# nasa/atmospheric-neural-rendering

Hardware: AMD Instinct MI355X
Metric: train-step rays/sec (higher is better)
Workload: dtype f16; 1 GPU; instant_ngp BASELINE configs[2]: 16-level T=2^19 hash grid, 2x64 fused MLP, 1024 samples/ray, full train step (fwd+loss+bwd+AdamW); global_batch=8192, per_rank_batch=8192, samples_per_ray=1024, parallelism=dp1

## Files before the change

### atmospheric-neural-rendering_amd/atmonr_amd/_lib.py

```python

from __future__ import annotations

import ctypes
import os
from ctypes import (
    POINTER,
    Structure,
    c_double,
    c_float,
    c_int32,
    c_int64,
    c_uint32,
    c_void_p,
)

import torch

_HERE = os.path.dirname(os.path.abspath(__file__))
LIB_PATH = os.environ.get("ANR_HIP_LIB", os.path.join(_HERE, "_native", "libanr_hip.so"))

F32, F16, BF16 = 0, 1, 2
MAX_LEVELS = 32

LOSS_CODES = {
# ... 240 lines not shown
         _P, _P, _P, c_int64, _P, c_int64, _P, _P, _P, c_int64, _P],
    ),
    "anr_occupancy_n_blocks": (c_int64, [c_int64]),
    "anr_occupancy_count": (
        c_int32, [_P, c_int64, _P, c_int32, c_int32, c_int32, c_float, _P, _P]),
    "anr_occupancy_compact": (
        c_int32, [_P, c_int64, _P, c_int32, c_int32, c_int32, c_float, _P, _P, _P, _P]),
    "anr_composite_force_generic": (c_int32, [c_int32]),
    "anr_composite_fwd": (
        c_int32,
        [_P, c_float, _P, _P, _P, c_int32, c_int64, c_int32, c_int32, c_int32,
         _P, _P, _P, _P, _P, _P],
    ),
    "anr_composite_bwd": (
        c_int32,
        [_P, c_float, _P, _P, _P, c_int32, c_int64, c_int32, c_int32, c_int32,
         _P, _P, _P, _P, _P, _P, _P, _P, _P, _P],
    ),
    "anr_loss_workspace_bytes": (c_int64, [c_int64]),
    "anr_loss_fwd_bwd": (
        c_int32,
        [c_int32, _P, c_int32, c_int32, _P, _P, c_int64, c_float, c_float, _P, _P, _P, _P],
    ),
    "anr_composite_ref16_set_rays": (c_int32, [c_int32]),
    "anr_composite_ref16_fwd": (
        c_int32,
        [_P, c_float, _P, _P, _P, c_int32, c_int64, c_int32, c_int32, _P, _P, _P, _P, _P, _P,
         _P, _P],
    ),
    "anr_composite_ref16_bwd": (
        c_int32,
        [_P, c_float, _P, _P, _P, c_int32, c_int64, c_int32, c_int32, _P, _P, _P, _P, c_int32,
         _P, _P],
    ),
    "anr_loss_ref16_fwd_bwd": (
        c_int32, [c_int32, _P, c_int32, _P, _P, c_int64, c_float, _P, _P, _P, _P]),
    "anr_grad_quantize_f16": (c_int32, [_P, c_int64, c_float, _P]),
    "anr_ingp_field_bwd_ref16": (
        c_int32,
        [POINTER(MlpDesc), POINTER(MlpDesc), _P, _P, c_int64, _P, c_int64, c_int64, _P, _P,
         c_int64, _P, c_int64, _P, _P, c_float, _P],
    ),
    "anr_ingp_field_bwd_ref16_tiles": (
        c_int32,
        [POINTER(MlpDesc), POINTER(MlpDesc), _P, _P, c_int64, _P, c_int64, c_int64, _P, _P,
         c_int64, _P, c_int64, _P, _P, c_float, _P, _P],
    ),
    "anr_ingp_field_bwd_ref16_rows": (
        c_int32,
        [POINTER(MlpDesc), POINTER(MlpDesc), _P, _P, c_int64, _P, c_int64, c_int64, _P, _P,
         c_int64, _P, c_int64, _P, _P, c_float, _P, _P, c_int64, _P],
    ),
    "anr_ingp_field_bwd_ref16_rows_h": (
        c_int32,
        [POINTER(MlpDesc), POINTER(MlpDesc), _P, _P, c_int64, _P, c_int64, c_int64, _P, _P,
         c_int64, _P, c_int64, _P, _P, c_float, _P, _P, c_int64, _P],
    ),
    "anr_ingp_field_bwd_ref16_rows_workspace_bytes": (c_int64, [c_int64]),
    "anr_mlp_bwd_ref16": (
        c_int32,
        [POINTER(MlpDesc), _P, _P, c_int32, c_int64, c_int64, _P, c_int32, c_int64, _P,
         c_int32, c_int64, _P, _P, c_int64, c_float, _P],
    ),
    "anr_adam_step": (
        c_int32,
        [_P, _P, _P, _P, _P, c_int64, c_float, c_float, c_float, c_float, c_float,
# ... 253 lines not shown
```

### atmospheric-neural-rendering_amd/atmonr_amd/graphics_utils.py

```python

from __future__ import annotations

import torch

from . import _lib
from ._lib import ANRError, call, dtype_code, ptr


class _CompositeFn(torch.autograd.Function):
    @staticmethod
    def forward(ctx, z, color, sigma, color_surf, z_scale: float, want_alpha: bool):
        B, N, C = color.shape
        S = sigma.shape[2]
        dt = color.dtype
        dev = color.device
        sigma = sigma.to(dt).contiguous()
        color = color.contiguous()
        cs = color_surf.to(dt).contiguous() if color_surf is not None else None
        zc = z.float().contiguous()
        color_map = torch.empty(B, C, device=dev, dtype=dt)
        atmo = torch.empty(B, C, device=dev, dtype=dt) if cs is not None else None
        surf = torch.empty(B, C, device=dev, dtype=dt) if cs is not None else None
        weights = torch.empty(B, N, S, device=dev, dtype=dt)
        alpha = torch.empty(B, N, S, device=dev, dtype=dt)
# ... 15 lines not shown
        B, N, C = color.shape
        S = sigma.shape[2]
        dt = color.dtype
        dev = color.device
        if ctx.has_surf:
            g_cm, g_alpha, g_w, g_atmo, g_surf = grads
        else:
            g_cm, g_alpha, g_w = grads
            g_atmo = g_surf = None

        def prep(g):
            return None if g is None else g.to(dt).contiguous()

        if g_cm is None:
            g_cm = torch.zeros(B, color.shape[2], device=dev, dtype=dt)

        need_z, need_c, need_s, need_cs = ctx.needs_input_grad[:4]
        d_color = torch.empty_like(color) if need_c else None
        d_sigma = torch.empty_like(sigma) if need_s else None
        d_cs = torch.empty_like(cs) if (need_cs and cs is not None) else None
        d_z = torch.empty(B, N, device=dev, dtype=torch.float32) if need_z else None
        args = (ptr(zc), ctx.z_scale, ptr(color), ptr(sigma), ptr(cs), dtype_code(dt), B, N, C,
                S, ptr(prep(g_cm)), ptr(prep(g_atmo)), ptr(prep(g_surf)), ptr(prep(g_w)),
                ptr(prep(g_alpha)), ptr(d_color), ptr(d_sigma), ptr(d_cs), ptr(d_z))
        call("anr_composite_bwd", *args, _lib.stream(dev))
        if d_z is not None:
            d_z = d_z.to(ctx.z_dtype)
        return d_z, d_color, d_sigma, d_cs, None, None


class _CompositeRef16Fn(torch.autograd.Function):

    @staticmethod
    def forward(ctx, z, color, sigma, color_surf, z_scale: float, zero_rays, want16: bool):
        B, N, C = color.shape
        if sigma.shape[2] != 1:
            raise ANRError("reference-numerics composite: one density channel (B, N, 1)")
        dev = color.device
        color, sigma = color.contiguous(), sigma.contiguous()
        cs = color_surf.to(color.dtype).contiguous() if color_surf is not None else None
        zc = z.float().contiguous()
        f16 = torch.float16
        cm = torch.empty(B, C, device=dev, dtype=f16)
        atmo = torch.empty(B, C, device=dev, dtype=f16)
        surf = torch.empty(B, C, device=dev, dtype=f16) if cs is not None else None
        weights = torch.empty(B, N, 1, device=dev, dtype=f16)
        alpha = torch.empty(B, N, 1, device=dev, dtype=f16)
        copies = want16 and color.dtype != f16
        c16 = torch.empty(B, N, C, device=dev, dtype=f16) if copies else None
        s16 = torch.empty(B, N, 1, device=dev, dtype=f16) if copies else None
        call("anr_composite_ref16_fwd", ptr(zc), float(z_scale), ptr(color), ptr(sigma), ptr(cs),
             dtype_code(color.dtype), B, N, C, ptr(cm), ptr(atmo), ptr(surf), ptr(weights),
             ptr(alpha), ptr(c16), ptr(s16), _lib.stream(dev), tag="composite_fwd")
        ctx.out_dtype = color.dtype
        if copies:
            ctx.save_for_backward(zc, c16, s16, cs)
        else:
            ctx.save_for_backward(zc, color, sigma, cs)
            if want16:
                c16, s16 = color.detach(), sigma.detach()
        ctx.set_materialize_grads(False)
        ctx.z_scale = float(z_scale)
        ctx.zero_rays = zero_rays
        outs = (cm, alpha, weights) if cs is None else (cm, alpha, weights, atmo, surf)
        if want16:
            ctx.mark_non_differentiable(c16, s16)
            outs = outs + (c16, s16)
        return outs

    @staticmethod
    def backward(ctx, g_cm, *unused):
        zc, color, sigma, cs = ctx.saved_tensors
        if any(g is not None for g in unused):
            raise ANRError("reference-numerics composite: gradients flow through color_map "
                           "only (as in the reference's loss)")
        B, N, C = color.shape
        dev = color.device
        if g_cm is None:
            g_cm = torch.zeros(B, C, device=dev, dtype=torch.float16)
        g_cm = g_cm.to(torch.float16).contiguous()
        od = ctx.out_dtype
        d_color = torch.empty(color.shape, device=dev, dtype=od)
        d_sigma = torch.empty(sigma.shape, device=dev, dtype=od)
        d_cs = (torch.empty(cs.shape, device=dev, dtype=od)
                if cs is not None and ctx.needs_input_grad[3] else None)
        if cs is not None and cs.dtype != color.dtype:
            cs = cs.to(color.dtype)
        call("anr_composite_ref16_bwd", ptr(zc), ctx.z_scale, ptr(color), ptr(sigma), ptr(cs),
             dtype_code(color.dtype), B, N, C, ptr(g_cm), ptr(d_color), ptr(d_sigma), ptr(d_cs),
             dtype_code(od), ptr(ctx.zero_rays), _lib.stream(dev), tag="composite_bwd")
        return None, d_color, d_sigma, d_cs, None, None, None


def render_with_surface_ref16(z_vals, color, sigma, color_surf, z_scale: float = 1.0,
                              zero_rays: torch.Tensor | None = None, inputs_f16: bool = False):
    _check(z_vals, color, sigma)
    if zero_rays is None:
        zero_rays = torch.zeros(1, dtype=torch.int32, device=color.device)
    return _CompositeRef16Fn.apply(z_vals, color, sigma, color_surf, z_scale, zero_rays,
                                   bool(inputs_f16))


def _check(z_vals, color, sigma):
    if not (z_vals.dim() == 2 and color.dim() == 3 and sigma.dim() == 3):
        raise ANRError("render: expected z (B,N), color (B,N,C), sigma (B,N,S)")
    if z_vals.shape != color.shape[:2] or z_vals.shape != sigma.shape[:2]:
        raise ANRError("render: z / color / sigma shapes disagree")
    if color.dtype not in (torch.float16, torch.float32):
        raise ANRError(f"render: unsupported dtype {color.dtype}")


def render(z_vals: torch.Tensor, color: torch.Tensor, sigma: torch.Tensor, z_scale: float = 1.0):
    _check(z_vals, color, sigma)
    return _CompositeFn.apply(z_vals, color, sigma, None, z_scale, True)


def render_with_surface(z_vals, color, sigma, color_surf, z_scale: float = 1.0):
    _check(z_vals, color, sigma)
    return _CompositeFn.apply(z_vals, color, sigma, color_surf, z_scale, True)
```

### atmospheric-neural-rendering_amd/atmonr_amd/pipelines/instant_ngp.py

```python

from __future__ import annotations

import os
from itertools import chain
from typing import Any, Mapping

import torch
import torch.nn.functional as F
from torch.optim import Optimizer

from .. import _lib
from ..field import IngpFieldFn, field_density, field_fused
from ..graphics_utils import render_with_surface, render_with_surface_ref16
from ..losses import LOSSES, indexed_loss, indexed_loss_ref16
from ..occupancy import OccupancyGrid, pipeline_density
from ..optim import FusedAdam
from ..samplers import (points_with_heights, preprocess_points, sample_and_preprocess,
                        sample_uniform_bins)
from ..tcnn import Encoding, Network
from .pipeline import Pipeline


class InstantNGPPipeline(Pipeline):
    module_names = ["pos_encoder", "pos_mlp", "dir_encoder", "dir_mlp", "surf_encoder",
# ... 139 lines not shown
                out = _lib.JoinAtBackwardEnd.apply(out, main)

        def join():
            main.wait_stream(side)
            out.record_stream(main)
            return out
        return join

    def _forward_fused(self, ray_batch, u=None):
        B = ray_batch["origin"].shape[0]
        N = self.config["num_samples_per_ray"]
        surf_branch = self._surface_async(ray_batch)
        _, z_vals, coords = sample_and_preprocess(ray_batch, N, self._prep_ngp, u=u)
        occ = self.occupancy
        if occ is not None and self.training:
            occ.update(pipeline_density(self))
        params = (self.pos_encoder.params, self.pos_mlp.params, self.dir_mlp.params, self)
        _lib.grad_use(*params[:3])
        if occ is not None and occ.active:
            rows, kept = occ.compact(coords.view(B * N, 3))
            sigma, color = IngpFieldFn.apply(kept, ray_batch["dir"].float(), N, *params, rows,
                                             B * N)
        else:
            sigma, color = IngpFieldFn.apply(coords.view(B * N, coords.shape[-1]),
                                             ray_batch["dir"].float(), N, *params)
        color = color.view(B, N, -1)
        sigma = sigma.view(B, N, 1)
        color_surf = surf_branch()
        if self.numerics == "reference":
            if self._zero_rays is None:
                self._zero_rays = torch.zeros(1, dtype=torch.int32, device=color.device)
            color_map, _, weights, atmo, surf, color, sigma = render_with_surface_ref16(
                z_vals, color, sigma, color_surf, z_scale=self.scale / 1000,
                zero_rays=self._zero_rays, inputs_f16=True)
            if color_map.requires_grad:
                color_map = _TcnnGradsAtBackwardEnd.apply(color_map, self)
        else:
            color_map, _, weights, atmo, surf = render_with_surface(
                z_vals, color, sigma, color_surf, z_scale=self.scale / 1000)
        results = {
            "color_fine": color[:, :-1],
            "color_surf": color_surf,
            "color_map_surf": surf,
            "color_map_atmo": atmo,
            "sigma_fine": sigma[:, :-1],
            "color_map_fine": color_map,
            "weights_fine": weights,
            "z_vals_fine": z_vals,
        }
        if self.include_height:
            results["norm_heights_fine"] = coords[..., 3]
        return results

    def _forward_reference(self, ray_batch, u=None):
        B_ = ray_batch["origin"].shape[0]
        N = self.config["num_samples_per_ray"]
        pts, z_vals = sample_uniform_bins(ray_batch, N, u=u)
        if self.point_preprocessor:
            pts = self.point_preprocessor(pts)
        pts = (pts + 1) / 2
        if self.include_height:
            pts = points_with_heights(pts, self._prep_height)
        dirs = ray_batch["dir"][:, None].repeat(1, N, 1)
        pts[..., 2] = pts[..., 2] / self.config["alt_compress_factor"]
        pos_enc = self.pos_encoder(pts.view(B_ * N, -1))
        pos_out = self.pos_mlp(pos_enc)
        dir_enc = self.dir_encoder(
# ... 108 lines not shown
```

### atmospheric-neural-rendering_amd/csrc/ref16.hip

```cpp
#pragma clang fp contract(off)

#include <stdlib.h>

#include <type_traits>

#include "anr_common.h"

namespace anr {
namespace ref16 {

constexpr int kMaxC = 8;
constexpr int kSeg = 64;

__device__ __forceinline__ float h(float x) {
  asm("" : "+v"(x));
  return __half2float(__float2half_rn(x));
}

__device__ __forceinline__ float h64(double d) {
  float f = static_cast<float>(d);
  if (static_cast<double>(f) != d && f != 0.0f && isfinite(f)) {
    uint32_t u = __float_as_uint(f);
    if (fabs(static_cast<double>(f)) > fabs(d)) u -= 1;
    f = __uint_as_float(u | 1u);
// ... 70 lines not shown
__device__ __forceinline__ Sample from_e(float e, float dl) {
  Sample s;
  s.delta = dl;
  s.e = e;
  s.alpha = h(1.0f - s.e);
  s.q2 = h(h(1.0f - s.alpha) + 1e-10f);
  return s;
}

__device__ __forceinline__ Sample sample(float sig, float dl) {
  const float x = h(-sig * dl);
  return from_e(h64(exp(static_cast<double>(x))), dl);
}

constexpr int kPad = 72;

template <int R>
struct __attribute__((aligned(16))) FwdLds {
  _Float16 q2[R][kPad];
  _Float16 alpha[R][kPad];
  _Float16 T[R][kPad];
  _Float16 t[kMaxC][R][kPad];
};
typedef _Float16 h8v __attribute__((ext_vector_type(8)));

__device__ __forceinline__ float mul_h(float a, _Float16 q) {
  return __builtin_fmaf(a, static_cast<float>(q), 0.0f);
}
__device__ __forceinline__ float add_h(float acc, _Float16 x) {
  return __builtin_fmaf(static_cast<float>(x), 1.0f, acc);
}
constexpr float kNegZero = -0.0f;

template <int R, typename T>
__global__ void __launch_bounds__(64) fwd_kernel(const float* __restrict__ z, float zs,
                                                 const T* __restrict__ color,
                                                 const T* __restrict__ sigma,
                                                 const T* __restrict__ cs, int64_t B, int N,
                                                 int C, __half* cmap, __half* atmo_out,
                                                 __half* surf_out, __half* weights,
                                                 __half* alpha_out, __half* color16,
                                                 __half* sigma16) {
  __shared__ FwdLds<R> L;
  const int64_t b0 = static_cast<int64_t>(blockIdx.x) * R;
  const int nr = B - b0 < R ? static_cast<int>(B - b0) : R;
  const int lane = threadIdx.x;
  const int sr = lane / C, sc = lane - sr * C;
  _Float16 cp = 1.0f;
  float pr = 1.0f;
  float acc = 0.0f;
  SegIn<R, true, true> nxt;
  nxt.fetch(z, sigma, color, b0, nr, 0, N, C, lane);
  for (int s0 = 0; s0 < N; s0 += kSeg) {
    const int n = N - s0 < kSeg ? N - s0 : kSeg;
    const int nv = (n + 7) & ~7;
    const SegIn<R, true, true> cur = nxt;
    if (s0 + kSeg < N) nxt.fetch(z, sigma, color, b0, nr, s0 + kSeg, N, C, lane);
#pragma unroll
    for (int r = 0; r < R; ++r) {
      if (r < nr && lane < n) {
        const int64_t b = b0 + r;
        const float sg = in16<T>(cur.sg[r]);
        if (sigma16) sigma16[b * N + s0 + lane] = __float2half_rn(sg);
        const Sample sm = sample(sg, delta_z(cur.zm[r], cur.z0[r], cur.zp[r], zs, s0 + lane, N));
        L.q2[r][lane] = static_cast<_Float16>(sm.q2);
        L.alpha[r][lane] = static_cast<_Float16>(sm.alpha);
      } else if (lane < nv) {
        L.q2[r][lane] = static_cast<_Float16>(1.0f);
      }
    }
    wave_sync();
    if (lane < nr) {
      for (int l8 = 0; l8 < nv; l8 += 8) {
        const h8v q = *reinterpret_cast<const h8v*>(&L.q2[lane][l8]);
        h8v tv;
#pragma unroll
        for (int k = 0; k < 8; ++k) {
          tv[k] = cp;
          cp = cp * q[k];
          pr = mul_h(pr, q[k]);
        }
        *reinterpret_cast<h8v*>(&L.T[lane][l8]) = tv;
      }
    }
    wave_sync();
#pragma unroll
    for (int r = 0; r < R; ++r) {
      if (r < nr && lane < n) {
        const int64_t i = (b0 + r) * N + s0 + lane;
        const float al = static_cast<float>(L.alpha[r][lane]);
        const float w = h(al * static_cast<float>(L.T[r][lane]));
#pragma unroll
        for (int c = 0; c < kMaxC; ++c) {
          if (c >= C) break;
          const float col = in16<T>(cur.col[r][c]);
          if (color16) color16[i * C + c] = __float2half_rn(col);
          L.t[c][r][lane] = static_cast<_Float16>(h(col * w));
        }
        if (weights) weights[i] = __float2half_rn(w);
        if (alpha_out) alpha_out[i] = __float2half_rn(al);
      } else if (lane < nv) {
        for (int c = 0; c < C; ++c) L.t[c][r][lane] = static_cast<_Float16>(kNegZero);
      }
    }
    wave_sync();
    if (sr < nr) {
      for (int l8 = 0; l8 < nv; l8 += 8) {
        const h8v tv = *reinterpret_cast<const h8v*>(&L.t[sc][sr][l8]);
#pragma unroll
        for (int k = 0; k < 8; ++k) acc = add_h(acc, tv[k]);
      }
    }
    wave_sync();
  }
  const float prr = h(__shfl(pr, sr < R ? sr : 0));
  if (sr < nr) {
    const int64_t b = b0 + sr;
    const int c = sc;
    const float atmo = h(acc);
    const float surf = cs ? h(prr * h(ld(cs, b * C + c))) : 0.0f;
    cmap[b * C + c] = __float2half_rn(cs ? h(atmo + surf) : atmo);
    if (atmo_out) atmo_out[b * C + c] = __float2half_rn(atmo);
    if (surf_out && cs) surf_out[b * C + c] = __float2half_rn(surf);
  }
}

template <int R>
struct __attribute__((aligned(16))) BwdLds {
  _Float16 q2[R][kPad];
  _Float16 u[R][kPad];
  _Float16 rin[R][kPad];
  float g[R][kMaxC];
  float g_pr[R];
  float pr[R];
};

template <int R, typename T, typename G>
__global__ void __launch_bounds__(64) bwd_kernel(const float* __restrict__ z, float zs,
                                                 const T* __restrict__ color,
                                                 const T* __restrict__ sigma,
                                                 const T* __restrict__ cs, int64_t B, int N,
                                                 int C, const __half* __restrict__ g_cm,
                                                 G* d_color, G* d_sigma, G* d_cs,
                                                 int* zero_rays) {
  __shared__ BwdLds<R> L;
  const int64_t b0 = static_cast<int64_t>(blockIdx.x) * R;
  const int nr = B - b0 < R ? static_cast<int>(B - b0) : R;
  const int lane = threadIdx.x;
  const int sr = lane / C, sc = lane - sr * C;
  constexpr bool GH = std::is_same<G, __half>::value;
  typedef uint32_t __attribute__((may_alias)) pair_t;
  const bool pair = GH && C >= 2 && ((static_cast<int64_t>(N) * C) & 1) == 0 &&
                    (reinterpret_cast<uintptr_t>(d_color) & 3) == 0;
  auto park = [&](int64_t b) { return reinterpret_cast<pair_t*>(d_color + b * N * C); };
  auto in = [](float x) {
    if constexpr (GH) return in16<T>(x);
    else return h(x);
  };
  const bool cvec = GH && color_vec4(color, C);
  float gl = 0.0f;
  if (sr < nr) {
    gl = __half2float(g_cm[(b0 + sr) * C + sc]);
    L.g[sr][sc] = gl;
  }
  _Float16 cp = 1.0f;
  float pr = 1.0f;
  uint32_t zmask = 0;
  SegIn<R, false, true> nxt;
  nxt.fetch(z, sigma, color, b0, nr, 0, N, C, lane);
  for (int s0 = 0; s0 < N; s0 += kSeg) {
    const int n = N - s0 < kSeg ? N - s0 : kSeg;
    const int nv = (n + 7) & ~7;
    const SegIn<R, false, true> cur = nxt;
    if (s0 + kSeg < N) nxt.fetch(z, sigma, color, b0, nr, s0 + kSeg, N, C, lane);
    float e1[R];
#pragma unroll
    for (int r = 0; r < R; ++r) {
      bool zr = false;
      e1[r] = 0.0f;
      if (r < nr && lane < n) {
        const int64_t b = b0 + r;
        const Sample sm = sample(in(cur.sg[r]),
                                 delta_z(cur.zm[r], cur.z0[r], cur.zp[r], zs, s0 + lane, N));
        L.q2[r][lane] = static_cast<_Float16>(sm.q2);
        e1[r] = sm.e;
        if (!(GH && pair)) d_color[(b * N + s0 + lane) * C] = static_cast<G>(sm.e);
        zr = sm.q2 == 0.0f;
      } else if (lane < nv) {
        L.q2[r][lane] = static_cast<_Float16>(1.0f);
      }
      if (__any(zr)) zmask |= 1u << r;
    }
    wave_sync();
    if (lane < nr) {
      for (int l8 = 0; l8 < nv; l8 += 8) {
        const h8v q = *reinterpret_cast<const h8v*>(&L.q2[lane][l8]);
        h8v tv;
#pragma unroll
        for (int k = 0; k < 8; ++k) {
          tv[k] = cp;
          cp = cp * q[k];
          pr = mul_h(pr, q[k]);
        }
        *reinterpret_cast<h8v*>(&L.u[lane][l8]) = tv;
      }
    }
    wave_sync();
#pragma unroll
    for (int r = 0; r < R; ++r)
      if (r < nr && lane < n) {
        if (GH && pair) {
          const uint32_t tb = __builtin_bit_cast(uint16_t, L.u[r][lane]);
          const uint32_t eb = __builtin_bit_cast(uint16_t, static_cast<_Float16>(e1[r]));
          park(b0 + r)[s0 + lane] = tb | (eb << 16);
        } else {
          d_sigma[(b0 + r) * N + s0 + lane] = static_cast<G>(static_cast<float>(L.u[r][lane]));
        }
      }
    wave_sync();
  }
  const float prr = h(__shfl(pr, sr < R ? sr : 0));
  if (lane < nr) L.pr[lane] = h(pr);
  if (cs && sr < nr) {
    if (d_cs) d_cs[(b0 + sr) * C + sc] = static_cast<G>(h(gl * prr));
  }
  if (lane < nr) {
    float g_pr = 0.0f;
    if (cs) {
      for (int c = 0; c < C; ++c) {
        const float csv = h(ld(cs, (b0 + lane) * C + c));
        g_pr = g_pr + h(L.g[lane][c] * csv);
      }
      g_pr = h(g_pr);
    }
    L.g_pr[lane] = g_pr;
  }
  if (zmask && lane == 0) atomicAdd(zero_rays, __popc(zmask));
  wave_sync();
  _Float16 rc = 0.0f;
  float zm_[R], z0_[R], zp_[R], ee_[R], tt_[R], col_[R][kMaxC];
  auto fetch2 = [&](int s0) {
    const int i = s0 + lane;
#pragma unroll
    for (int r = 0; r < R; ++r) {
      if (r < nr && lane < N - s0) {
        const int64_t k = (b0 + r) * N + i;
        const float* zr = z + (b0 + r) * N;
        z0_[r] = zr[i];
        zm_[r] = i > 0 ? zr[i - 1] : 0.0f;
        zp_[r] = i < N - 1 ? zr[i + 1] : 0.0f;
        if constexpr (GH) {
          uint32_t pv;
          if (pair) {
            pv = park(b0 + r)[i];
          } else {
            const uint32_t tb = __builtin_bit_cast(uint16_t, d_sigma[k]);
            const uint32_t eb = __builtin_bit_cast(uint16_t, d_color[k * C]);
            pv = tb | (eb << 16);
          }
          tt_[r] = static_cast<float>(__builtin_bit_cast(_Float16, static_cast<uint16_t>(pv)));
          ee_[r] = static_cast<float>(__builtin_bit_cast(_Float16, static_cast<uint16_t>(pv >> 16)));
        } else {
          ee_[r] = static_cast<float>(d_color[k * C]);
          tt_[r] = static_cast<float>(d_sigma[k]);
        }
        h4v v = {0, 0, 0, 0};
        if (GH && cvec) v = *reinterpret_cast<const h4v*>(color + k * 4);
#pragma unroll
        for (int c = 0; c < kMaxC; ++c)
          if (c < C && !(GH && cvec)) col_[r][c] = ld(color, k * C + c);
        if constexpr (GH) {
#pragma unroll
          for (int c = 0; c < 4; ++c)
            if (cvec) col_[r][c] = static_cast<float>(v[c]);
        }
      }
    }
  };
  fetch2(((N - 1) / kSeg) * kSeg);
  wave_sync();
  for (int s0 = ((N - 1) / kSeg) * kSeg; s0 >= 0; s0 -= kSeg) {
    const int n = N - s0 < kSeg ? N - s0 : kSeg;
    const int nv = (n + 7) & ~7;
    float czm[R], cz0[R], czp[R], cee[R], ctt[R], ccol[R][kMaxC];
// ... 181 lines not shown
    const bool two = type == ANR_LOSS_L1_PLUS_HDR || type == ANR_LOSS_MSE_PLUS_HDR;
    *loss = two ? h(v1 + h(v2 * 0.2f)) : v1;
  }
}

__global__ void __launch_bounds__(256) quantize_kernel(float* __restrict__ g, int64_t n,
                                                       float s, float inv_s) {
  const int64_t stride = static_cast<int64_t>(gridDim.x) * blockDim.x;
  for (int64_t i = static_cast<int64_t>(blockIdx.x) * blockDim.x + threadIdx.x; i < n;
       i += stride)
    g[i] = h(h(g[i] * s) * inv_s);
}

static int g_rays = 0;
static int rays_per_wave(int C, int64_t B) {
  int R = g_rays ? g_rays : (B >= 8192 ? 2 : 1);
  while (R > 1 && R * C > 64) R /= 2;
  return R;
}

}
}

using namespace anr;

extern "C" int anr_composite_ref16_set_rays(int32_t rays_per_wave) {
  ANR_CHECK_ARG(rays_per_wave == 0 || rays_per_wave == 1 || rays_per_wave == 2 ||
                    rays_per_wave == 4 || rays_per_wave == 8,
                "anr_composite_ref16_set_rays: %d (0 = default, 1 / 2 / 4 / 8)", rays_per_wave);
  ref16::g_rays = rays_per_wave;
  return ANR_OK;
}

extern "C" int anr_composite_ref16_fwd(const float* z, float z_scale, const void* color,
                                       const void* sigma, const void* color_surf,
                                       int32_t in_dtype, int64_t B, int32_t N, int32_t C,
                                       void* color_map, void* color_map_atmo,
                                       void* color_map_surf, void* weights, void* alpha,
                                       void* color16, void* sigma16, anr_stream_t stream) {
  ANR_CHECK_ARG(z && color && sigma && color_map, "anr_composite_ref16_fwd: null argument");
  ANR_CHECK_ARG(B >= 0 && N >= 1 && C >= 1 && C <= ref16::kMaxC,
                "anr_composite_ref16_fwd: bad shape B=%lld N=%d C=%d", (long long)B, N, C);
  ANR_CHECK_ARG(in_dtype == ANR_F16 || in_dtype == ANR_F32, "anr_composite_ref16_fwd: bad dtype");
  if (B == 0) return ANR_OK;
  ANR_CHECK_ARG(B < (1LL << 31), "anr_composite_ref16_fwd: B=%lld too large", (long long)B);
  const int R = ref16::rays_per_wave(C, B);
#define ANR_R16F(RR, T)                                                                        \
  hipLaunchKernelGGL((ref16::fwd_kernel<RR, T>), dim3(static_cast<unsigned>(ceil_div(B, RR))), \
                     dim3(64), 0, as_stream(stream), z, z_scale,                               \
                     static_cast<const T*>(color), static_cast<const T*>(sigma),               \
                     static_cast<const T*>(color_surf), B, N, C,                              \
                     static_cast<__half*>(color_map), static_cast<__half*>(color_map_atmo),  \
                     static_cast<__half*>(color_map_surf), static_cast<__half*>(weights),     \
                     static_cast<__half*>(alpha), static_cast<__half*>(color16),              \
                     static_cast<__half*>(sigma16))
#define ANR_R16F_T(T)                                                                         \
  switch (R) {                                                                                \
    case 1: ANR_R16F(1, T); break;                                                            \
    case 2: ANR_R16F(2, T); break;                                                            \
    case 4: ANR_R16F(4, T); break;                                                            \
    default: ANR_R16F(8, T); break;                                                           \
  }
  if (in_dtype == ANR_F16) { ANR_R16F_T(__half) } else { ANR_R16F_T(float) }
#undef ANR_R16F_T
#undef ANR_R16F
  ANR_CHECK_LAUNCH("anr_composite_ref16_fwd");
  return ANR_OK;
}

extern "C" int anr_composite_ref16_bwd(const float* z, float z_scale, const void* color,
                                       const void* sigma, const void* color_surf,
                                       int32_t in_dtype, int64_t B, int32_t N, int32_t C,
                                       const void* d_color_map, void* d_color, void* d_sigma,
                                       void* d_color_surf, int32_t out_dtype, int32_t* zero_rays,
                                       anr_stream_t stream) {
  ANR_CHECK_ARG(z && color && sigma && d_color_map && d_color && d_sigma && zero_rays,
                "anr_composite_ref16_bwd: null argument");
  ANR_CHECK_ARG(B >= 0 && N >= 1 && C >= 1 && C <= ref16::kMaxC,
                "anr_composite_ref16_bwd: bad shape");
  ANR_CHECK_ARG(in_dtype == ANR_F16 || in_dtype == ANR_F32, "anr_composite_ref16_bwd: bad dtype");
  ANR_CHECK_ARG(out_dtype == ANR_F16 || out_dtype == ANR_F32,
                "anr_composite_ref16_bwd: bad output dtype");
  ANR_CHECK_ARG(d_color_surf == nullptr || color_surf != nullptr,
                "anr_composite_ref16_bwd: d_color_surf without color_surf");
  if (B == 0) return ANR_OK;
  ANR_CHECK_ARG(B < (1LL << 31), "anr_composite_ref16_bwd: B=%lld too large", (long long)B);
  const int R = ref16::rays_per_wave(C, B);
#define ANR_R16B(RR, T, G)                                                                     \
  hipLaunchKernelGGL((ref16::bwd_kernel<RR, T, G>),                                           \
                     dim3(static_cast<unsigned>(ceil_div(B, RR))), dim3(64), 0,               \
                     as_stream(stream), z, z_scale,                                           \
                     static_cast<const T*>(color), static_cast<const T*>(sigma),               \
                     static_cast<const T*>(color_surf), B, N, C,                              \
                     static_cast<const __half*>(d_color_map), static_cast<G*>(d_color),       \
                     static_cast<G*>(d_sigma), static_cast<G*>(d_color_surf), zero_rays)
#define ANR_R16B_TG(T, G)                                                                     \
  switch (R) {                                                                                \
    case 1: ANR_R16B(1, T, G); break;                                                         \
    case 2: ANR_R16B(2, T, G); break;                                                         \
    case 4: ANR_R16B(4, T, G); break;                                                         \
    default: ANR_R16B(8, T, G); break;                                                        \
  }
  if (in_dtype == ANR_F16) {
    if (out_dtype == ANR_F16) { ANR_R16B_TG(__half, __half) } else { ANR_R16B_TG(__half, float) }
  } else {
    if (out_dtype == ANR_F16) { ANR_R16B_TG(float, __half) } else { ANR_R16B_TG(float, float) }
  }
#undef ANR_R16B_TG
#undef ANR_R16B
  ANR_CHECK_LAUNCH("anr_composite_ref16_bwd");
  return ANR_OK;
}

extern "C" int anr_loss_ref16_fwd_bwd(int32_t loss_type, const void* color_map, int32_t C,
                                      const int64_t* irgb_idx, const float* gt, int64_t B,
                                      float max_i, float* loss_out, void* grad_out,
                                      void* workspace, anr_stream_t stream) {
  ANR_CHECK_ARG(color_map && irgb_idx && gt && loss_out && workspace,
                "anr_loss_ref16_fwd_bwd: null argument");
  ANR_CHECK_ARG(loss_type >= ANR_LOSS_DARK && loss_type <= ANR_LOSS_MSE_PLUS_HDR,
                "anr_loss_ref16_fwd_bwd: unknown loss %d", loss_type);
  ANR_CHECK_ARG(B >= 1 && C >= 1, "anr_loss_ref16_fwd_bwd: bad shape");
  const int nblk = static_cast<int>(ceil_div(B, 256));
  const float inv = 1.0f / max_i;
  const float eps = static_cast<float>(1e-3 * static_cast<double>(max_i));
  const float norm = __half2float(__float2half_rn(static_cast<float>(2.0 / static_cast<double>(B))));
  const float inv_n = static_cast<float>(1.0 / static_cast<double>(B));
  hipLaunchKernelGGL(ref16::loss_kernel, dim3(nblk), dim3(256), 0, as_stream(stream), loss_type,
                     static_cast<const __half*>(color_map), C, irgb_idx, gt, B, inv, eps, norm,
                     inv_n, static_cast<__half*>(grad_out), static_cast<float*>(workspace));
  ANR_CHECK_LAUNCH("anr_loss_ref16_fwd_bwd");
  hipLaunchKernelGGL(ref16::loss_finalize_kernel, dim3(1), dim3(64), 0, as_stream(stream),
                     loss_type, static_cast<const float*>(workspace), nblk, B, loss_out);
  ANR_CHECK_LAUNCH("anr_loss_ref16_fwd_bwd(finalize)");
  return ANR_OK;
}

extern "C" int anr_grad_quantize_f16(float* grad, int64_t n, float loss_scale,
                                     anr_stream_t stream) {
  ANR_CHECK_ARG(grad != nullptr || n == 0, "anr_grad_quantize_f16: null argument");
  ANR_CHECK_ARG(n >= 0 && loss_scale > 0.0f, "anr_grad_quantize_f16: bad argument");
  if (n == 0) return ANR_OK;
  int64_t blocks = ceil_div(n, 256);
  if (blocks > 8192) blocks = 8192;
// ... 6 lines not shown
```

### include/anr.h

```cpp
#ifndef ANR_H_
#define ANR_H_

#include <stdint.h>

#ifdef __cplusplus
extern "C" {
#endif

#define ANR_ABI_VERSION 5

enum anr_dtype { ANR_F32 = 0, ANR_F16 = 1, ANR_BF16 = 2 };

enum anr_status {
  ANR_OK = 0,
  ANR_E_INVALID = -1,
  ANR_E_LAUNCH = -2,
  ANR_E_UNSUPPORTED = -3
};

typedef void* anr_stream_t;

int anr_abi_version(void);
const char* anr_last_error(void);

// ... 233 lines not shown

int anr_composite_fwd(const float* z, float z_scale, const void* color, const void* sigma,
                      const void* color_surf, int32_t io_dtype, int64_t B, int32_t N,
                      int32_t C, int32_t S, void* color_map, void* color_map_atmo,
                      void* color_map_surf, void* weights, void* alpha,
                      anr_stream_t stream);
int anr_composite_force_generic(int32_t on);
int anr_composite_bwd(const float* z, float z_scale, const void* color, const void* sigma,
                      const void* color_surf, int32_t io_dtype, int64_t B, int32_t N,
                      int32_t C, int32_t S, const void* d_color_map, const void* d_atmo,
                      const void* d_surf, const void* d_weights, const void* d_alpha,
                      void* d_color, void* d_sigma, void* d_color_surf, float* d_z,
                      anr_stream_t stream);

enum anr_loss { ANR_LOSS_DARK = 0, ANR_LOSS_HDR = 1, ANR_LOSS_L1 = 2,
                ANR_LOSS_L1_PLUS_HDR = 3, ANR_LOSS_MSE = 4, ANR_LOSS_MSE_PLUS_HDR = 5 };
int64_t anr_loss_workspace_bytes(int64_t B);
int anr_loss_fwd_bwd(int32_t loss_type, const void* color_map, int32_t pred_dtype,
                     int32_t C, const int64_t* irgb_idx, const float* gt, int64_t B,
                     float max_i, float grad_scale, float* loss_out, void* grad_out,
                     void* workspace, anr_stream_t stream);

int anr_composite_ref16_set_rays(int32_t rays_per_wave);
int anr_composite_ref16_fwd(const float* z, float z_scale, const void* color,
                            const void* sigma, const void* color_surf, int32_t in_dtype,
                            int64_t B, int32_t N, int32_t C, void* color_map,
                            void* color_map_atmo, void* color_map_surf, void* weights,
                            void* alpha, void* color16, void* sigma16, anr_stream_t stream);
int anr_composite_ref16_bwd(const float* z, float z_scale, const void* color,
                            const void* sigma, const void* color_surf, int32_t in_dtype,
                            int64_t B, int32_t N, int32_t C, const void* d_color_map,
                            void* d_color, void* d_sigma, void* d_color_surf,
                            int32_t out_dtype, int32_t* zero_rays, anr_stream_t stream);
int anr_loss_ref16_fwd_bwd(int32_t loss_type, const void* color_map, int32_t C,
                           const int64_t* irgb_idx, const float* gt, int64_t B, float max_i,
                           float* loss_out, void* grad_out, void* workspace,
                           anr_stream_t stream);
int anr_grad_quantize_f16(float* grad, int64_t n, float loss_scale, anr_stream_t stream);
int anr_ingp_field_bwd_ref16(const anr_mlp_desc* pos, const anr_mlp_desc* dir,
                             const void* packed, const void* enc, int64_t enc_stride,
                             const float* dirs, int64_t n_per_ray, int64_t M,
                             const float* d_sigma, const float* d_color,
                             int64_t d_color_stride, float* d_enc, int64_t d_enc_stride,
                             float* g_pos, float* g_dir, float loss_scale,
                             anr_stream_t stream);
int anr_ingp_field_bwd_ref16_tiles(const anr_mlp_desc* pos, const anr_mlp_desc* dir,
                                   const void* packed, const void* enc, int64_t enc_stride,
                                   const float* dirs, int64_t n_per_ray, int64_t M,
                                   const float* d_sigma, const float* d_color,
                                   int64_t d_color_stride, float* d_enc, int64_t d_enc_stride,
                                   float* g_pos, float* g_dir, float loss_scale,
                                   uint8_t* tile_nz, anr_stream_t stream);
int64_t anr_ingp_field_bwd_ref16_rows_workspace_bytes(int64_t M);
int anr_ingp_field_bwd_ref16_rows(const anr_mlp_desc* pos, const anr_mlp_desc* dir,
                                  const void* packed, const void* enc, int64_t enc_stride,
                                  const float* dirs, int64_t n_per_ray, int64_t M,
                                  const float* d_sigma, const float* d_color,
                                  int64_t d_color_stride, void* d_enc_h, int64_t d_enc_stride,
                                  float* g_pos, float* g_dir, float loss_scale,
                                  uint32_t* row_nz, void* workspace, int64_t workspace_bytes,
                                  anr_stream_t stream);
int anr_ingp_field_bwd_ref16_rows_h(const anr_mlp_desc* pos, const anr_mlp_desc* dir,
                                    const void* packed, const void* enc, int64_t enc_stride,
                                    const float* dirs, int64_t n_per_ray, int64_t M,
                                    const void* d_sigma, const void* d_color,
                                    int64_t d_color_stride, void* d_enc_h, int64_t d_enc_stride,
// ... 42 lines not shown
```

Baseline: 4.900 million rays/s.

## Park forward transmittance and exp terms for composite backward; skip alpha output

The forward composite kernel now optionally writes a packed per-sample word (f16 transmittance plus f16 exp term) and a per-ray word (final transmittance plus zero flag). The backward kernel reads these instead of rerunning the whole forward scan over z, sigma and color, which removes a full sequential pass over all samples. The instant-NGP pipeline also stops materialising the alpha output. The cost is an extra B*N int32 buffer written in forward and held until backward, which adds memory traffic and footprint.

```diff
diff --git a/atmospheric-neural-rendering_amd/atmonr_amd/_lib.py b/atmospheric-neural-rendering_amd/atmonr_amd/_lib.py
--- a/atmospheric-neural-rendering_amd/atmonr_amd/_lib.py
+++ b/atmospheric-neural-rendering_amd/atmonr_amd/_lib.py
@@ -296,6 +296,16 @@
         c_int32,
         [_P, c_float, _P, _P, _P, c_int32, c_int64, c_int32, c_int32, _P, _P, _P, _P, c_int32,
          _P, _P],
+    ),
+    "anr_composite_ref16_fwd_park": (
+        c_int32,
+        [_P, c_float, _P, _P, _P, c_int32, c_int64, c_int32, c_int32, _P, _P, _P, _P, _P, _P,
+         _P, _P, _P, _P],
+    ),
+    "anr_composite_ref16_bwd_parked": (
+        c_int32,
+        [_P, c_float, _P, _P, _P, c_int32, c_int64, c_int32, c_int32, _P, _P, _P, _P, c_int32,
+         _P, _P, _P, _P],
     ),
     "anr_loss_ref16_fwd_bwd": (
         c_int32, [c_int32, _P, c_int32, _P, _P, c_int64, c_float, _P, _P, _P, _P]),
diff --git a/atmospheric-neural-rendering_amd/atmonr_amd/graphics_utils.py b/atmospheric-neural-rendering_amd/atmonr_amd/graphics_utils.py
--- a/atmospheric-neural-rendering_amd/atmonr_amd/graphics_utils.py
+++ b/atmospheric-neural-rendering_amd/atmonr_amd/graphics_utils.py
@@ -71,7 +71,8 @@
 class _CompositeRef16Fn(torch.autograd.Function):
 
     @staticmethod
-    def forward(ctx, z, color, sigma, color_surf, z_scale: float, zero_rays, want16: bool):
+    def forward(ctx, z, color, sigma, color_surf, z_scale: float, zero_rays, want16: bool,
+                need_alpha: bool, park: bool):
         B, N, C = color.shape
         if sigma.shape[2] != 1:
             raise ANRError("reference-numerics composite: one density channel (B, N, 1)")
@@ -84,18 +85,27 @@
         atmo = torch.empty(B, C, device=dev, dtype=f16)
         surf = torch.empty(B, C, device=dev, dtype=f16) if cs is not None else None
         weights = torch.empty(B, N, 1, device=dev, dtype=f16)
-        alpha = torch.empty(B, N, 1, device=dev, dtype=f16)
+        alpha = torch.empty(B, N, 1, device=dev, dtype=f16) if need_alpha else None
         copies = want16 and color.dtype != f16
         c16 = torch.empty(B, N, C, device=dev, dtype=f16) if copies else None
         s16 = torch.empty(B, N, 1, device=dev, dtype=f16) if copies else None
-        call("anr_composite_ref16_fwd", ptr(zc), float(z_scale), ptr(color), ptr(sigma), ptr(cs),
-             dtype_code(color.dtype), B, N, C, ptr(cm), ptr(atmo), ptr(surf), ptr(weights),
-             ptr(alpha), ptr(c16), ptr(s16), _lib.stream(dev), tag="composite_fwd")
+        args = (ptr(zc), float(z_scale), ptr(color), ptr(sigma), ptr(cs),
+                dtype_code(color.dtype), B, N, C, ptr(cm), ptr(atmo), ptr(surf), ptr(weights),
+                ptr(alpha), ptr(c16), ptr(s16))
+        if park:
+            pk = torch.empty(B, N, device=dev, dtype=torch.int32)
+            rpk = torch.empty(B, device=dev, dtype=torch.int32)
+            call("anr_composite_ref16_fwd_park", *args, ptr(pk), ptr(rpk), _lib.stream(dev),
+                 tag="composite_fwd")
+        else:
+            pk = rpk = None
+            call("anr_composite_ref16_fwd", *args, _lib.stream(dev), tag="composite_fwd")
         ctx.out_dtype = color.dtype
+        ctx.parked = park
         if copies:
-            ctx.save_for_backward(zc, c16, s16, cs)
+            ctx.save_for_backward(zc, c16, s16, cs, pk, rpk)
         else:
-            ctx.save_for_backward(zc, color, sigma, cs)
+            ctx.save_for_backward(zc, color, sigma, cs, pk, rpk)
             if want16:
                 c16, s16 = color.detach(), sigma.detach()
         ctx.set_materialize_grads(False)
@@ -109,7 +119,7 @@
 
     @staticmethod
     def backward(ctx, g_cm, *unused):
-        zc, color, sigma, cs = ctx.saved_tensors
+        zc, color, sigma, cs, pk, rpk = ctx.saved_tensors
         if any(g is not None for g in unused):
             raise ANRError("reference-numerics composite: gradients flow through color_map "
                            "only (as in the reference's loss)")
@@ -125,19 +135,27 @@
                 if cs is not None and ctx.needs_input_grad[3] else None)
         if cs is not None and cs.dtype != color.dtype:
             cs = cs.to(color.dtype)
-        call("anr_composite_ref16_bwd", ptr(zc), ctx.z_scale, ptr(color), ptr(sigma), ptr(cs),
-             dtype_code(color.dtype), B, N, C, ptr(g_cm), ptr(d_color), ptr(d_sigma), ptr(d_cs),
-             dtype_code(od), ptr(ctx.zero_rays), _lib.stream(dev), tag="composite_bwd")
-        return None, d_color, d_sigma, d_cs, None, None, None
+        args = (ptr(zc), ctx.z_scale, ptr(color), ptr(sigma), ptr(cs), dtype_code(color.dtype),
+                B, N, C, ptr(g_cm), ptr(d_color), ptr(d_sigma), ptr(d_cs), dtype_code(od),
+                ptr(ctx.zero_rays))
+        if pk is not None:
+            call("anr_composite_ref16_bwd_parked", *args, ptr(pk), ptr(rpk), _lib.stream(dev),
+                 tag="composite_bwd")
+        else:
+            call("anr_composite_ref16_bwd", *args, _lib.stream(dev), tag="composite_bwd")
+        return None, d_color, d_sigma, d_cs, None, None, None, None, None
 
 
 def render_with_surface_ref16(z_vals, color, sigma, color_surf, z_scale: float = 1.0,
-                              zero_rays: torch.Tensor | None = None, inputs_f16: bool = False):
+                              zero_rays: torch.Tensor | None = None, inputs_f16: bool = False,
+                              need_alpha: bool = True):
     _check(z_vals, color, sigma)
     if zero_rays is None:
         zero_rays = torch.zeros(1, dtype=torch.int32, device=color.device)
+    park = torch.is_grad_enabled() and any(
+        t is not None and t.requires_grad for t in (color, sigma, color_surf))
     return _CompositeRef16Fn.apply(z_vals, color, sigma, color_surf, z_scale, zero_rays,
-                                   bool(inputs_f16))
+                                   bool(inputs_f16), bool(need_alpha), park)
 
 
 def _check(z_vals, color, sigma):
diff --git a/atmospheric-neural-rendering_amd/atmonr_amd/pipelines/instant_ngp.py b/atmospheric-neural-rendering_amd/atmonr_amd/pipelines/instant_ngp.py
--- a/atmospheric-neural-rendering_amd/atmonr_amd/pipelines/instant_ngp.py
+++ b/atmospheric-neural-rendering_amd/atmonr_amd/pipelines/instant_ngp.py
@@ -195,7 +195,7 @@
                 self._zero_rays = torch.zeros(1, dtype=torch.int32, device=color.device)
             color_map, _, weights, atmo, surf, color, sigma = render_with_surface_ref16(
                 z_vals, color, sigma, color_surf, z_scale=self.scale / 1000,
-                zero_rays=self._zero_rays, inputs_f16=True)
+                zero_rays=self._zero_rays, inputs_f16=True, need_alpha=False)
             if color_map.requires_grad:
                 color_map = _TcnnGradsAtBackwardEnd.apply(color_map, self)
         else:
diff --git a/atmospheric-neural-rendering_amd/csrc/ref16.hip b/atmospheric-neural-rendering_amd/csrc/ref16.hip
--- a/atmospheric-neural-rendering_amd/csrc/ref16.hip
+++ b/atmospheric-neural-rendering_amd/csrc/ref16.hip
@@ -126,7 +126,14 @@
 }
 constexpr float kNegZero = -0.0f;
 
-template <int R, typename T>
+__device__ __forceinline__ uint32_t f16_bits(float x) {
+  return __builtin_bit_cast(uint16_t, static_cast<_Float16>(x));
+}
+__device__ __forceinline__ float f16_value(uint32_t bits) {
+  return static_cast<float>(__builtin_bit_cast(_Float16, static_cast<uint16_t>(bits)));
+}
+
+template <int R, typename T, bool PARK>
 __global__ void __launch_bounds__(64) fwd_kernel(const float* __restrict__ z, float zs,
                                                  const T* __restrict__ color,
                                                  const T* __restrict__ sigma,
@@ -134,7 +141,8 @@
                                                  int C, __half* cmap, __half* atmo_out,
                                                  __half* surf_out, __half* weights,
                                                  __half* alpha_out, __half* color16,
-                                                 __half* sigma16) {
+                                                 __half* sigma16, uint32_t* park,
+                                                 uint32_t* ray_park) {
   __shared__ FwdLds<R> L;
   const int64_t b0 = static_cast<int64_t>(blockIdx.x) * R;
   const int nr = B - b0 < R ? static_cast<int>(B - b0) : R;
@@ -143,6 +151,7 @@
   _Float16 cp = 1.0f;
   float pr = 1.0f;
   float acc = 0.0f;
+  uint32_t zmask = 0;
   SegIn<R, true, true> nxt;
   nxt.fetch(z, sigma, color, b0, nr, 0, N, C, lane);
   for (int s0 = 0; s0 < N; s0 += kSeg) {
@@ -150,8 +159,11 @@
     const int nv = (n + 7) & ~7;
     const SegIn<R, true, true> cur = nxt;
     if (s0 + kSeg < N) nxt.fetch(z, sigma, color, b0, nr, s0 + kSeg, N, C, lane);
+    uint32_t eb[R];
 #pragma unroll
     for (int r = 0; r < R; ++r) {
+      bool zr = false;
+      eb[r] = 0;
       if (r < nr && lane < n) {
         const int64_t b = b0 + r;
         const float sg = in16<T>(cur.sg[r]);
@@ -159,9 +171,14 @@
         const Sample sm = sample(sg, delta_z(cur.zm[r], cur.z0[r], cur.zp[r], zs, s0 + lane, N));
         L.q2[r][lane] = static_cast<_Float16>(sm.q2);
         L.alpha[r][lane] = static_cast<_Float16>(sm.alpha);
+        if (PARK) {
+          eb[r] = f16_bits(sm.e) << 16;
+          zr = sm.q2 == 0.0f;
+        }
       } else if (lane < nv) {
         L.q2[r][lane] = static_cast<_Float16>(1.0f);
       }
+      if (PARK && __any(zr)) zmask |= 1u << r;
     }
     wave_sync();
     if (lane < nr) {
@@ -183,7 +200,9 @@
       if (r < nr && lane < n) {
         const int64_t i = (b0 + r) * N + s0 + lane;
         const float al = static_cast<float>(L.alpha[r][lane]);
-        const float w = h(al * static_cast<float>(L.T[r][lane]));
+        const _Float16 Ti = L.T[r][lane];
+        const float w = h(al * static_cast<float>(Ti));
+        if (PARK) park[i] = __builtin_bit_cast(uint16_t, Ti) | eb[r];
 #pragma unroll
         for (int c = 0; c < kMaxC; ++c) {
           if (c >= C) break;
@@ -217,6 +236,7 @@
     if (atmo_out) atmo_out[b * C + c] = __float2half_rn(atmo);
     if (surf_out && cs) surf_out[b * C + c] = __float2half_rn(surf);
   }
+  if (PARK && lane < nr) ray_park[b0 + lane] = f16_bits(h(pr)) | (((zmask >> lane) & 1u) << 16);
 }
 
 template <int R>
@@ -229,14 +249,16 @@
   float pr[R];
 };
 
-template <int R, typename T, typename G>
+template <int R, typename T, typename G, bool PARKED>
 __global__ void __launch_bounds__(64) bwd_kernel(const float* __restrict__ z, float zs,
                                                  const T* __restrict__ color,
                                                  const T* __restrict__ sigma,
                                                  const T* __restrict__ cs, int64_t B, int N,
                                                  int C, const __half* __restrict__ g_cm,
                                                  G* d_color, G* d_sigma, G* d_cs,
-                                                 int* zero_rays) {
+                                                 int* zero_rays,
+                                                 const uint32_t* __restrict__ pk,
+                                                 const uint32_t* __restrict__ ray_pk) {
   __shared__ BwdLds<R> L;
   const int64_t b0 = static_cast<int64_t>(blockIdx.x) * R;
   const int nr = B - b0 < R ? static_cast<int>(B - b0) : R;
@@ -261,8 +283,8 @@
   float pr = 1.0f;
   uint32_t zmask = 0;
   SegIn<R, false, true> nxt;
-  nxt.fetch(z, sigma, color, b0, nr, 0, N, C, lane);
-  for (int s0 = 0; s0 < N; s0 += kSeg) {
+  if (!PARKED) nxt.fetch(z, sigma, color, b0, nr, 0, N, C, lane);
+  for (int s0 = 0; s0 < (PARKED ? 0 : N); s0 += kSeg) {
     const int n = N - s0 < kSeg ? N - s0 : kSeg;
     const int nv = (n + 7) & ~7;
     const SegIn<R, false, true> cur = nxt;
@@ -313,8 +335,14 @@
       }
     wave_sync();
   }
-  const float prr = h(__shfl(pr, sr < R ? sr : 0));
-  if (lane < nr) L.pr[lane] = h(pr);
+  float prh = h(pr);
+  if (PARKED) {
+    const uint32_t rp = lane < nr ? ray_pk[b0 + lane] : 0u;
+    prh = f16_value(rp);
+    zmask = static_cast<uint32_t>(__ballot((rp >> 16) & 1u));
+  }
+  const float prr = __shfl(prh, sr < R ? sr : 0);
+  if (lane < nr) L.pr[lane] = prh;
   if (cs && sr < nr) {
     if (d_cs) d_cs[(b0 + sr) * C + sc] = static_cast<G>(h(gl * prr));
   }
@@ -343,7 +371,11 @@
         z0_[r] = zr[i];
         zm_[r] = i > 0 ? zr[i - 1] : 0.0f;
         zp_[r] = i < N - 1 ? zr[i + 1] : 0.0f;
-        if constexpr (GH) {
+        if constexpr (PARKED) {
+          const uint32_t pv = pk[k];
+          tt_[r] = f16_value(pv);
+          ee_[r] = f16_value(pv >> 16);
+        } else if constexpr (GH) {
           uint32_t pv;
           if (pair) {
             pv = park(b0 + r)[i];
@@ -591,12 +623,12 @@
   return ANR_OK;
 }
 
-extern "C" int anr_composite_ref16_fwd(const float* z, float z_scale, const void* color,
-                                       const void* sigma, const void* color_surf,
-                                       int32_t in_dtype, int64_t B, int32_t N, int32_t C,
-                                       void* color_map, void* color_map_atmo,
-                                       void* color_map_surf, void* weights, void* alpha,
-                                       void* color16, void* sigma16, anr_stream_t stream) {
+static int composite_ref16_fwd(const float* z, float z_scale, const void* color,
+                               const void* sigma, const void* color_surf, int32_t in_dtype,
+                               int64_t B, int32_t N, int32_t C, void* color_map,
+                               void* color_map_atmo, void* color_map_surf, void* weights,
+                               void* alpha, void* color16, void* sigma16, uint32_t* park,
+                               uint32_t* ray_park, anr_stream_t stream) {
   ANR_CHECK_ARG(z && color && sigma && color_map, "anr_composite_ref16_fwd: null argument");
   ANR_CHECK_ARG(B >= 0 && N >= 1 && C >= 1 && C <= ref16::kMaxC,
                 "anr_composite_ref16_fwd: bad shape B=%lld N=%d C=%d", (long long)B, N, C);
@@ -604,36 +636,65 @@
   if (B == 0) return ANR_OK;
   ANR_CHECK_ARG(B < (1LL << 31), "anr_composite_ref16_fwd: B=%lld too large", (long long)B);
   const int R = ref16::rays_per_wave(C, B);
-#define ANR_R16F(RR, T)                                                                        \
-  hipLaunchKernelGGL((ref16::fwd_kernel<RR, T>), dim3(static_cast<unsigned>(ceil_div(B, RR))), \
+#define ANR_R16F(RR, T, P)                                                                     \
+  hipLaunchKernelGGL((ref16::fwd_kernel<RR, T, P>),                                            \
+                     dim3(static_cast<unsigned>(ceil_div(B, RR))),                             \
                      dim3(64), 0, as_stream(stream), z, z_scale,                               \
                      static_cast<const T*>(color), static_cast<const T*>(sigma),               \
                      static_cast<const T*>(color_surf), B, N, C,                              \
                      static_cast<__half*>(color_map), static_cast<__half*>(color_map_atmo),  \
                      static_cast<__half*>(color_map_surf), static_cast<__half*>(weights),     \
                      static_cast<__half*>(alpha), static_cast<__half*>(color16),              \
-                     static_cast<__half*>(sigma16))
-#define ANR_R16F_T(T)                                                                         \
+                     static_cast<__half*>(sigma16), park, ray_park)
+#define ANR_R16F_T(T, P)                                                                      \
   switch (R) {                                                                                \
-    case 1: ANR_R16F(1, T); break;                                                            \
-    case 2: ANR_R16F(2, T); break;                                                            \
-    case 4: ANR_R16F(4, T); break;                                                            \
-    default: ANR_R16F(8, T); break;                                                           \
-  }
-  if (in_dtype == ANR_F16) { ANR_R16F_T(__half) } else { ANR_R16F_T(float) }
+    case 1: ANR_R16F(1, T, P); break;                                                         \
+    case 2: ANR_R16F(2, T, P); break;                                                         \
+    case 4: ANR_R16F(4, T, P); break;                                                         \
+    default: ANR_R16F(8, T, P); break;                                                        \
+  }
+  if (park) {
+    if (in_dtype == ANR_F16) { ANR_R16F_T(__half, true) } else { ANR_R16F_T(float, true) }
+  } else {
+    if (in_dtype == ANR_F16) { ANR_R16F_T(__half, false) } else { ANR_R16F_T(float, false) }
+  }
 #undef ANR_R16F_T
 #undef ANR_R16F
   ANR_CHECK_LAUNCH("anr_composite_ref16_fwd");
   return ANR_OK;
 }
 
-extern "C" int anr_composite_ref16_bwd(const float* z, float z_scale, const void* color,
+extern "C" int anr_composite_ref16_fwd(const float* z, float z_scale, const void* color,
                                        const void* sigma, const void* color_surf,
                                        int32_t in_dtype, int64_t B, int32_t N, int32_t C,
-                                       const void* d_color_map, void* d_color, void* d_sigma,
-                                       void* d_color_surf, int32_t out_dtype, int32_t* zero_rays,
-                                       anr_stream_t stream) {
-  ANR_CHECK_ARG(z && color && sigma && d_color_map && d_color && d_sigma && zero_rays,
+                                       void* color_map, void* color_map_atmo,
+                                       void* color_map_surf, void* weights, void* alpha,
+                                       void* color16, void* sigma16, anr_stream_t stream) {
+  return composite_ref16_fwd(z, z_scale, color, sigma, color_surf, in_dtype, B, N, C, color_map,
+                             color_map_atmo, color_map_surf, weights, alpha, color16, sigma16,
+                             nullptr, nullptr, stream);
+}
+
+extern "C" int anr_composite_ref16_fwd_park(const float* z, float z_scale, const void* color,
+                                            const void* sigma, const void* color_surf,
+                                            int32_t in_dtype, int64_t B, int32_t N, int32_t C,
+                                            void* color_map, void* color_map_atmo,
+                                            void* color_map_surf, void* weights, void* alpha,
+                                            void* color16, void* sigma16, uint32_t* park,
+                                            uint32_t* ray_park, anr_stream_t stream) {
+  ANR_CHECK_ARG(park && ray_park, "anr_composite_ref16_fwd_park: null park");
+  return composite_ref16_fwd(z, z_scale, color, sigma, color_surf, in_dtype, B, N, C, color_map,
+                             color_map_atmo, color_map_surf, weights, alpha, color16, sigma16,
+                             park, ray_park, stream);
+}
+
+static int composite_ref16_bwd(const float* z, float z_scale, const void* color,
+                               const void* sigma, const void* color_surf, int32_t in_dtype,
+                               int64_t B, int32_t N, int32_t C, const void* d_color_map,
+                               void* d_color, void* d_sigma, void* d_color_surf,
+                               int32_t out_dtype, int32_t* zero_rays, const uint32_t* park,
+                               const uint32_t* ray_park, anr_stream_t stream) {
+  ANR_CHECK_ARG(z && color && (sigma || park) && d_color_map && d_color && d_sigma && zero_rays,
                 "anr_composite_ref16_bwd: null argument");
   ANR_CHECK_ARG(B >= 0 && N >= 1 && C >= 1 && C <= ref16::kMaxC,
                 "anr_composite_ref16_bwd: bad shape");
@@ -645,30 +706,62 @@
   if (B == 0) return ANR_OK;
   ANR_CHECK_ARG(B < (1LL << 31), "anr_composite_ref16_bwd: B=%lld too large", (long long)B);
   const int R = ref16::rays_per_wave(C, B);
-#define ANR_R16B(RR, T, G)                                                                     \
-  hipLaunchKernelGGL((ref16::bwd_kernel<RR, T, G>),                                           \
+#define ANR_R16B(RR, T, G, P)                                                                  \
+  hipLaunchKernelGGL((ref16::bwd_kernel<RR, T, G, P>),                                        \
                      dim3(static_cast<unsigned>(ceil_div(B, RR))), dim3(64), 0,               \
                      as_stream(stream), z, z_scale,                                           \
                      static_cast<const T*>(color), static_cast<const T*>(sigma),               \
                      static_cast<const T*>(color_surf), B, N, C,                              \
                      static_cast<const __half*>(d_color_map), static_cast<G*>(d_color),       \
-                     static_cast<G*>(d_sigma), static_cast<G*>(d_color_surf), zero_rays)
-#define ANR_R16B_TG(T, G)                                                                     \
+                     static_cast<G*>(d_sigma), static_cast<G*>(d_color_surf), zero_rays,      \
+                     park, ray_park)
+#define ANR_R16B_TG(T, G, P)                                                                  \
   switch (R) {                                                                                \
-    case 1: ANR_R16B(1, T, G); break;                                                         \
-    case 2: ANR_R16B(2, T, G); break;                                                         \
-    case 4: ANR_R16B(4, T, G); break;                                                         \
-    default: ANR_R16B(8, T, G); break;                                                        \
-  }
-  if (in_dtype == ANR_F16) {
-    if (out_dtype == ANR_F16) { ANR_R16B_TG(__half, __half) } else { ANR_R16B_TG(__half, float) }
-  } else {
-    if (out_dtype == ANR_F16) { ANR_R16B_TG(float, __half) } else { ANR_R16B_TG(float, float) }
-  }
+    case 1: ANR_R16B(1, T, G, P); break;                                                      \
+    case 2: ANR_R16B(2, T, G, P); break;                                                      \
+    case 4: ANR_R16B(4, T, G, P); break;                                                      \
+    default: ANR_R16B(8, T, G, P); break;                                                     \
+  }
+#define ANR_R16B_P(P)                                                                         \
+  if (in_dtype == ANR_F16) {                                                                  \
+    if (out_dtype == ANR_F16) { ANR_R16B_TG(__half, __half, P) }                              \
+    else { ANR_R16B_TG(__half, float, P) }                                                    \
+  } else {                                                                                    \
+    if (out_dtype == ANR_F16) { ANR_R16B_TG(float, __half, P) }                               \
+    else { ANR_R16B_TG(float, float, P) }                                                     \
+  }
+  if (park) { ANR_R16B_P(true) } else { ANR_R16B_P(false) }
+#undef ANR_R16B_P
 #undef ANR_R16B_TG
 #undef ANR_R16B
   ANR_CHECK_LAUNCH("anr_composite_ref16_bwd");
   return ANR_OK;
+}
+
+extern "C" int anr_composite_ref16_bwd(const float* z, float z_scale, const void* color,
+                                       const void* sigma, const void* color_surf,
+                                       int32_t in_dtype, int64_t B, int32_t N, int32_t C,
+                                       const void* d_color_map, void* d_color, void* d_sigma,
+                                       void* d_color_surf, int32_t out_dtype, int32_t* zero_rays,
+                                       anr_stream_t stream) {
+  ANR_CHECK_ARG(sigma, "anr_composite_ref16_bwd: null argument");
+  return composite_ref16_bwd(z, z_scale, color, sigma, color_surf, in_dtype, B, N, C,
+                             d_color_map, d_color, d_sigma, d_color_surf, out_dtype, zero_rays,
+                             nullptr, nullptr, stream);
+}
+
+extern "C" int anr_composite_ref16_bwd_parked(const float* z, float z_scale, const void* color,
+                                              const void* sigma, const void* color_surf,
+                                              int32_t in_dtype, int64_t B, int32_t N, int32_t C,
+                                              const void* d_color_map, void* d_color,
+                                              void* d_sigma, void* d_color_surf,
+                                              int32_t out_dtype, int32_t* zero_rays,
+                                              const uint32_t* park, const uint32_t* ray_park,
+                                              anr_stream_t stream) {
+  ANR_CHECK_ARG(park && ray_park, "anr_composite_ref16_bwd_parked: null park");
+  return composite_ref16_bwd(z, z_scale, color, sigma, color_surf, in_dtype, B, N, C,
+                             d_color_map, d_color, d_sigma, d_color_surf, out_dtype, zero_rays,
+                             park, ray_park, stream);
 }
 
 extern "C" int anr_loss_ref16_fwd_bwd(int32_t loss_type, const void* color_map, int32_t C,
diff --git a/include/anr.h b/include/anr.h
--- a/include/anr.h
+++ b/include/anr.h
@@ -289,6 +289,19 @@
                             int64_t B, int32_t N, int32_t C, const void* d_color_map,
                             void* d_color, void* d_sigma, void* d_color_surf,
                             int32_t out_dtype, int32_t* zero_rays, anr_stream_t stream);
+int anr_composite_ref16_fwd_park(const float* z, float z_scale, const void* color,
+                                 const void* sigma, const void* color_surf, int32_t in_dtype,
+                                 int64_t B, int32_t N, int32_t C, void* color_map,
+                                 void* color_map_atmo, void* color_map_surf, void* weights,
+                                 void* alpha, void* color16, void* sigma16, uint32_t* park,
+                                 uint32_t* ray_park, anr_stream_t stream);
+int anr_composite_ref16_bwd_parked(const float* z, float z_scale, const void* color,
+                                   const void* sigma, const void* color_surf,
+                                   int32_t in_dtype, int64_t B, int32_t N, int32_t C,
+                                   const void* d_color_map, void* d_color, void* d_sigma,
+                                   void* d_color_surf, int32_t out_dtype, int32_t* zero_rays,
+                                   const uint32_t* park, const uint32_t* ray_park,
+                                   anr_stream_t stream);
 int anr_loss_ref16_fwd_bwd(int32_t loss_type, const void* color_map, int32_t C,
                            const int64_t* irgb_idx, const float* gt, int64_t B, float max_i,
                            float* loss_out, void* grad_out, void* workspace,
```

Measured after the change: 5.069 million rays/s, median of 6. 1.03x the previous value.
